# angelvillar96/STLPose

Measured on AMD Instinct MI355X. Metric: images/sec/GPU HRNet-W32 384x288 train step; PCKh@0.5 parity, higher is better.
Workload: dtype f16/bf16; 1 GPU; HRNet-W32 384x288 bs=32/GPU train step (fwd+MSE+bwd+Adam), random-init weights; global_batch=32, parallelism=dp1

## Files before the change

### stlpose_amd/csrc/wgrad.hip

```cpp
#include <type_traits>
#include "common.cuh"

#ifndef STL_DT
#define STL_DT 2
#endif

constexpr int WG_MAXG = STL_WGRAD_GROUP_MAX;
struct WgK {
    stl_wgrad p;
    stl_wgrad_io io[WG_MAXG];
    int ng;
    int dbg;
    int tiles_c, npt, HR, HC, HP, PI, pad, taps;
    int psg, psh;
    int off_cg, off_ch, off_g, off_h;
    float r_TW, r_HC, r_tc, r_vp, r_PI;
    unsigned long long m_tc, m_vp, m_PI;
    int xmap, units, gy, gz;
};

int stl_wgrad_backend_bf16(bool wide, const WgK& k, dim3 grid, size_t lds, hipStream_t st);
int stl_wgrad_backend_f32(bool wide, const WgK& k, dim3 grid, size_t lds, hipStream_t st);

namespace {

#include "conv_common.inc"

#ifdef STL_STAMPS
#include "../../include/stlpose_hip_debug.h"
__device__ long long g_wstamps[16];
__device__ long long g_wstamps2[64];
#define WSTAMP(i)                                                                                   \
    do {                                                                                            \
        if (k.dbg && blockIdx.x == 0 && blockIdx.y == 0 && blockIdx.z == 0 && threadIdx.x == 0) g_wstamps[i] = wall_clock64(); \
    } while (0)
#define WSTAMP2(i)                                                                                  \
    do {                                                                                            \
        if (k.dbg && blockIdx.x == 0 && blockIdx.y == 0 && blockIdx.z == 0 && threadIdx.x == 0 && (i) < 64) g_wstamps2[i] = wall_clock64(); \
    } while (0)
#else
#define WSTAMP(i) do {} while (0)
#define WSTAMP2(i) do {} while (0)
#endif

__device__ __forceinline__ int mad24_vsv(int a, int b_uniform, int c) {
    int r;
    asm("v_mad_i32_i24 %0, %1, %2, %3" : "=v"(r) : "v"(a), "s"(b_uniform), "v"(c));
    return r;
}

__device__ __forceinline__ int sdiv(int n, unsigned long long m) { return (int)(((unsigned long long)(uint32_t)n * m) >> 32); }


struct WgBlock { int member, bsplit, cy, cz; bool live; };
__device__ __forceinline__ WgBlock wg_block(const WgK& k) {
    WgBlock b;
    if (!k.xmap) {
        b.member = __builtin_amdgcn_readfirstlane(blockIdx.x / k.p.nsplit);
        b.bsplit = blockIdx.x - b.member * k.p.nsplit, b.cy = blockIdx.y, b.cz = blockIdx.z, b.live = true;
        return b;
    }
    const int nc = k.gy * k.gz, xcd = blockIdx.x & 7, j = blockIdx.x >> 3;
    const int ju = __builtin_amdgcn_readfirstlane(j / nc), chunk = j - ju * nc, unit = ju * 8 + xcd;
    b.live = unit < k.units;
    b.member = __builtin_amdgcn_readfirstlane(unit / k.p.nsplit), b.bsplit = unit - b.member * k.p.nsplit;
    b.cy = __builtin_amdgcn_readfirstlane(chunk / k.gz), b.cz = chunk - b.cy * k.gz;
    return b;
}


__device__ __forceinline__ int krow16(int g, int i, int lane) { return 16 * (g >> 1) + 8 * i + 4 * (g & 1) + ((lane & 15) >> 2); }

template <typename T>
__device__ __forceinline__ V16 frag_tr(const char* base, const int* rowoff, int colbyte, int lane);
template <>
__device__ __forceinline__ V16 frag_tr<__bf16>(const char* base, const int* rowoff, int colbyte, int lane) {
    V16 v;
#pragma unroll
    for (int h = 0; h < 2; ++h) {
        const char* ptr = base + rowoff[h] + colbyte + (lane & 3) * 8;
        s16x4 r = __builtin_amdgcn_ds_read_tr16_b64_v4i16(
            (__attribute__((address_space(3))) s16x4*)(uintptr_t)(uint32_t)(uintptr_t)ptr);
        const uint64_t bits = __builtin_bit_cast(uint64_t, r);
        v.w[2 * h] = (uint32_t)bits;
        v.w[2 * h + 1] = (uint32_t)(bits >> 32);
    }
    return v;
}
template <>
__device__ __forceinline__ V16 frag_tr<float>(const char* base, const int* rowoff, int colbyte, int lane) {
    V16 v;
#pragma unroll
    for (int s = 0; s < 4; ++s)
        v.w[s] = *reinterpret_cast<const uint32_t*>(base + rowoff[s] + colbyte + (lane & 15) * 4);
    return v;
}

template <typename T>
__device__ __forceinline__ V16 frag_at(const uint32_t* addr, int off);
template <>
__device__ __forceinline__ V16 frag_at<__bf16>(const uint32_t* addr, int off) {
    V16 v;
#pragma unroll
    for (int h = 0; h < 2; ++h) {
        s16x4 r = __builtin_amdgcn_ds_read_tr16_b64_v4i16((__attribute__((address_space(3))) s16x4*)(uintptr_t)(addr[h] + off));
        const uint64_t bits = __builtin_bit_cast(uint64_t, r);
        v.w[2 * h] = (uint32_t)bits;
        v.w[2 * h + 1] = (uint32_t)(bits >> 32);
    }
    return v;
}
template <>
__device__ __forceinline__ V16 frag_at<float>(const uint32_t* addr, int off) {
    V16 v;
#pragma unroll
    for (int s = 0; s < 4; ++s) v.w[s] = *(const __attribute__((address_space(3))) uint32_t*)(uintptr_t)(addr[s] + off);
    return v;
}

template <typename T, int KS, int NVH, bool GQ, int TPX, int OCC, int NW, typename TY = T, int CH = 32, int NSET = 2>
__global__ __launch_bounds__(64 * NW, OCC) void wgrad_kernel(const WgK k) {
    extern __shared__ __attribute__((aligned(16))) char smem[];
    constexpr int KV = ET<T>::KV, TAPS = KS * KS;
    constexpr int KSTEP = 4 * KV;
    constexpr int NR = sizeof(T) == 2 ? 2 : 4;
    constexpr int VPX = CH / KV;
    constexpr int NT = 64 * NW;
    constexpr int NVG = TPX * VPX / NT;
    static_assert(NVG >= 1 && NVG * NT == TPX * VPX, "g staging slots must tile the block");
    constexpr int QW = CH / 16, WPG = QW * QW;
    static_assert((CH == 32 || CH == 64) && NW % WPG == 0 && (NSET == 1 || NSET == 2), "channel tile / wave count");
    constexpr int NTG = NW / WPG;
    constexpr int TPG = (TAPS + NTG - 1) / NTG;
    constexpr int PS = CH * (int)sizeof(T) + (sizeof(T) == 2 ? 32 : 16);
    constexpr int NKT = TPX / KSTEP;
    const stl_wgrad& p = k.p;
    const WgBlock wb = wg_block(k);
    if (!wb.live) return;
    const int member = wb.member, bsplit = wb.bsplit;
    const stl_wgrad_io& io = k.io[member];
    const int tid = threadIdx.x, lane = tid & 63, wave = tid >> 6, g = lane >> 4;
    const int mt = (wave % WPG) / QW, nt = wave % QW, tg = wave / WPG;
    const int co0 = wb.cy * CH, ci0 = wb.cz * CH;
    WSTAMP(0);
    float* cgc = reinterpret_cast<float*>(smem + k.off_cg);
    float* chc = reinterpret_cast<float*>(smem + k.off_ch);
    char* sG = smem + k.off_g;
    char* sH = smem + k.off_h;

    const int tilepx = p.TH * p.TW;
    const int vpitch = p.Ho + 1;
    const int hrow = k.HC * PS;

    int g_yx[NVG];
    const int g_part = tid % VPX;
#pragma unroll
    for (int i = 0; i < NVG; ++i) {
        const int m = (tid + i * NT) / VPX;
        g_yx[i] = -1;
        if (m < tilepx) {
            const int ty = fdiv(m, k.r_TW);
            g_yx[i] = (ty << 16) | (m - ty * p.TW);
        }
    }
    int h_rc[NVH];
#pragma unroll
    for (int i = 0; i < NVH; ++i) {
        const int v = tid + i * NT;
        h_rc[i] = -1;
        if (v < k.HP * VPX) {
            const int hp = v / VPX, hr = fdiv(hp, k.r_HC);
            h_rc[i] = (hr << 16) | (hp - hr * k.HC);
        }
    }
    const bool g_chok = (co0 + g_part * KV) < p.Co, h_chok = (ci0 + g_part * KV) < p.Ci;

    const uint32_t lterm = sizeof(T) == 2 ? (lane & 3) * 8 : (lane & 15) * 4;
    uint32_t gaw[NR], hbw[NKT][NR];
#pragma unroll
    for (int i = 0; i < NR; ++i) {
        const int c = sizeof(T) == 2 ? krow16(g, i, lane) : 4 * g + i;
        gaw[i] = (uint32_t)(uintptr_t)sG + c * PS + lterm + mt * 16 * (int)sizeof(T);
#pragma unroll
        for (int s = 0; s < NKT; ++s) {
            int m = s * KSTEP + c;
            if (m >= tilepx) m = 0;
            const int ty = fdiv(m, k.r_TW), tx = m - ty * p.TW;
            hbw[s][i] = (uint32_t)(uintptr_t)sH + ((ty * p.stride) * k.HC + tx * p.stride) * PS + lterm + nt * 16 * (int)sizeof(T);
        }
    }

    V16 rgv[NSET][NVG], rgq[NSET][GQ ? NVG : 1], rhv[NSET][NVH];
    uint32_t okm[NSET] = {};

    const int g_cbytes = p.Co * (int)sizeof(T), h_cbytes = p.Ci * (int)sizeof(T);
    const int g_wrap = -p.Wo * g_cbytes, h_wrap = (p.Hi - k.PI) * p.Wi * h_cbytes;
    const int n_vp = -vpitch, n_PI = -k.PI;
    uint32_t g_lo[NVG], h_lo[NVH], slot_ok = 0;
#pragma unroll
    for (int i = 0; i < NVG; ++i) {
        g_lo[i] = (uint32_t)(((g_yx[i] >> 16) * p.Wo + (g_yx[i] & 0xffff)) * g_cbytes + (co0 + g_part * KV) * (int)sizeof(T));
        if (g_yx[i] >= 0 && g_chok) slot_ok |= 1u << i;
    }
#pragma unroll
    for (int i = 0; i < NVH; ++i) {
        h_lo[i] = (uint32_t)(((h_rc[i] >> 16) * p.Wi + (h_rc[i] & 0xffff)) * h_cbytes + (ci0 + g_part * KV) * (int)sizeof(T));
        if (h_rc[i] >= 0 && h_chok) slot_ok |= 1u << (NVG + i);
    }
    auto tile_offsets = [&](int t, uint32_t* go, uint32_t* ho) __attribute__((always_inline)) -> uint32_t {
        const int tr = sdiv(t, k.m_tc), tc = t - tr * k.tiles_c;
        const int vr0 = tr * p.TH, c0 = tc * p.TW;
        const int gb0 = sdiv(vr0, k.m_vp), gy0 = vr0 - gb0 * vpitch;
        const uint32_t g_t = (uint32_t)(((vr0 - gb0) * p.Wo + c0) * g_cbytes);
        uint32_t ok = 0;
#pragma unroll
        for (int i = 0; i < NVG; ++i) {
            const int oy0 = gy0 + (g_yx[i] >> 16), c = c0 + (g_yx[i] & 0xffff);
            const int wr_ = fdiv(oy0 < 0 ? 0 : oy0, k.r_vp);
            const int oy = mad24_vsv(wr_, n_vp, oy0);
            const bool in = ((slot_ok >> i) & 1u) & (gb0 + wr_ < p.B) & (oy < p.Ho) & (c < p.Wo);
            go[i] = in ? (uint32_t)mad24_vsv(wr_, g_wrap, (int)(g_t + g_lo[i])) : 0u;
            ok |= in ? 1u << i : 0u;
        }
        const int vrs = vr0 * p.stride, cb = c0 * p.stride - k.pad;
        const int hb0 = sdiv(vrs, k.m_PI), hy0 = vrs - hb0 * k.PI - k.pad;
        const uint32_t h_t = (uint32_t)(((hb0 * p.Hi + hy0) * p.Wi + cb) * h_cbytes);
#pragma unroll
        for (int i = 0; i < NVH; ++i) {
            const int iy0 = hy0 + (h_rc[i] >> 16), ix = cb + (h_rc[i] & 0xffff);
            const int wr_ = fdiv(iy0 < 0 ? 0 : iy0, k.r_PI);
            const int iy = mad24_vsv(wr_, n_PI, iy0);
            const bool in = ((slot_ok >> (NVG + i)) & 1u) & (iy0 >= 0) & (ix >= 0) & (ix < p.Wi) & (hb0 + wr_ < p.B) & (iy < p.Hi);
            ho[i] = in ? (uint32_t)mad24_vsv(wr_, h_wrap, (int)(h_t + h_lo[i])) : 0u;
            ok |= in ? 1u << (NVG + i) : 0u;
        }
        return ok;
    };
    auto load_set = [&](auto SET, const uint32_t* go, const uint32_t* ho, uint32_t ok) __attribute__((always_inline)) {
        constexpr int S = decltype(SET)::value;
#pragma unroll
        for (int i = 0; i < NVG; ++i) {
            rgv[S][i] = ldg16((const char*)io.g.x + go[i]);
            if (GQ) rgq[S][i] = ldg16((const char*)io.g.y + go[i]);
        }
#pragma unroll
        for (int i = 0; i < NVH; ++i) rhv[S][i] = ldg16((const char*)io.h.x + ho[i]);
        okm[S] = ok;
    };
    auto fetch = [&](auto SET, int t) __attribute__((always_inline)) {
        uint32_t go[NVG], ho[NVH];
        const uint32_t ok = tile_offsets(t, go, ho);
        load_set(SET, go, ho, ok);
    };
    const float relu_lo = io.h.relu ? 0.f : -INFINITY;
    auto write_lds = [&](auto SET) __attribute__((always_inline)) {
        constexpr int S = decltype(SET)::value;
        const int cl = g_part * KV;
#pragma unroll
        for (int i = 0; i < NVG; ++i) {
            V16 val = rgv[S][i];
            if (GQ) val = xform_bnbwd<T, TY>(val, rgq[S][i], cgc + cl, cgc + CH + cl, cgc + 2 * CH + cl);
            mask16(val, (okm[S] >> i) & 1u);
            const int v = tid + i * NT;
            *reinterpret_cast<V16*>(sG + (v / VPX) * PS + g_part * 16) = val;
        }
#pragma unroll
        for (int i = 0; i < NVH; ++i) {
            V16 val = rhv[S][i];
            if (io.h.mode == STL_SRC_BN) val = xform_bn<T, TY>(val, chc + cl, chc + CH + cl, relu_lo);
            else val = xform_cvt<T, TY>(val);
            mask16(val, (okm[S] >> (NVG + i)) & 1u);
            const int v = tid + i * NT;
            if (h_rc[i] >= 0) *reinterpret_cast<V16*>(sH + (v / VPX) * PS + g_part * 16) = val;
        }
    };

    f32x4 acc[TPG];
#pragma unroll
    for (int t = 0; t < TPG; ++t) acc[t] = f32x4{0.f, 0.f, 0.f, 0.f};

    auto mfma_taps = [&](auto TAP0, auto NTAP) __attribute__((always_inline)) {
        constexpr int T0 = decltype(TAP0)::value, NTP = decltype(NTAP)::value;
        constexpr int NJ = NKT * NTP, PF = NTP >= 4 ? (CH == 64 ? 4 : 6) : 2;
        uint32_t ga[NR], hb[NKT][NR];
#pragma unroll
        for (int i = 0; i < NR; ++i) {
            ga[i] = gaw[i];
            asm volatile("" : "+v"(ga[i]));
#pragma unroll
            for (int s = 0; s < NKT; ++s) {
                hb[s][i] = hbw[s][i];
                asm volatile("" : "+v"(hb[s][i]));
            }
        }
        V16 aq[2], bq[PF];
        auto bfrag = [&](int j) __attribute__((always_inline)) {
            const int s = j / NTP, tap = T0 + j % NTP;
            uint32_t ad[NR];
#pragma unroll
            for (int i = 0; i < NR; ++i) ad[i] = hb[s][i] + (tap / KS) * hrow;
            return frag_at<T>(ad, (tap % KS) * PS);
        };
        aq[0] = frag_at<T>(ga, 0);
#pragma unroll
        for (int j = 0; j < PF - 1 && j < NJ; ++j) bq[j] = bfrag(j);
#pragma unroll
        for (int j = 0; j < NJ; ++j) {
            const int s = j / NTP, jt = j % NTP;
            if (jt == 0 && s + 1 < NKT) aq[(s + 1) & 1] = frag_at<T>(ga, (s + 1) * KSTEP * PS);
            if (j + PF - 1 < NJ) bq[(j + PF - 1) % PF] = bfrag(j + PF - 1);
            mma16<T>(acc[jt], aq[s & 1], bq[j % PF]);
        }
    };
    auto mfma_tile = [&]() __attribute__((always_inline)) {
        if constexpr (NTG == 1) {
            mfma_taps(std::integral_constant<int, 0>{}, std::integral_constant<int, TAPS>{});
        } else {
            if (tg == 0) mfma_taps(std::integral_constant<int, 0>{}, std::integral_constant<int, TPG>{});
            else mfma_taps(std::integral_constant<int, TPG>{}, std::integral_constant<int, TAPS - TPG>{});
        }
    };

    const int step = p.nsplit;
    int t = bsplit;
    WSTAMP(1);
    SrcRaw raw;
    const int cidx = tid - (256 - 2 * CH);
    const bool cw = cidx >= 0 && cidx < 2 * CH, cg = cidx < CH;
    const int cch = cidx & (CH - 1);
    const bool cok = cw && (cg ? co0 + cch < p.Co : ci0 + cch < p.Ci);
    if (cok) {
        if (cg) src_raw_load(io.g, co0 + cch, p.Co, raw);
        else src_raw_load(io.h, ci0 + cch, p.Ci, raw);
    }
    constexpr std::integral_constant<int, 0> I0{};
    constexpr std::integral_constant<int, 1> I1{};
    if (t < k.npt) fetch(I0, t);
    if constexpr (NSET == 2) {
        if (t + step < k.npt) fetch(I1, t + step);
    }
    WSTAMP(2);
    if (cw) {
        float a = 0.f, b = 0.f, cc = 0.f;
        if (cok) {
            if (cg) src_raw_finish(io.g, raw, a, b, cc);
            else src_raw_finish(io.h, raw, a, b, cc);
        }
        if (cg) cgc[cch] = a, cgc[CH + cch] = b, cgc[2 * CH + cch] = cc;
        else chc[cch] = a, chc[CH + cch] = b;
    }
    __syncthreads();
    WSTAMP(3);
    bool first = true;
    [[maybe_unused]] int dbg_i = 0;
    auto body = [&](auto SET) __attribute__((always_inline)) {
        WSTAMP2(4 * dbg_i);
        write_lds(SET);
        __syncthreads();
        WSTAMP2(4 * dbg_i + 1);
        if (first) WSTAMP(4);
        if (t + NSET * step < k.npt) fetch(SET, t + NSET * step);
        WSTAMP2(4 * dbg_i + 2);
        mfma_tile();
        __syncthreads();
        WSTAMP2(4 * dbg_i + 3);
#ifdef STL_STAMPS
        ++dbg_i;
#endif
        if (first) WSTAMP(5);
        first = false;
        t += step;
    };
    while (t < k.npt) {
        body(I0);
        if constexpr (NSET == 2) {
            if (t >= k.npt) break;
            body(I1);
        }
    }
    WSTAMP(6);
    {
        float* slab = io.partial + (size_t)bsplit * p.Co * TAPS * p.Ci;
        const int ci = ci0 + nt * 16 + (lane & 15), co = co0 + mt * 16 + 4 * g;
        const int tap0 = tg * TPG;
        float* dst = slab + ((size_t)co * TAPS + tap0) * p.Ci + ci;
        if (ci < p.Ci) {
#pragma unroll
            for (int jt = 0; jt < TPG; ++jt)
#pragma unroll
                for (int r = 0; r < 4; ++r)
                    if (tap0 + jt < TAPS && co + r < p.Co) dst[((size_t)r * TAPS + jt) * p.Ci] = acc[jt][r];
        }
    }
    WSTAMP(8);
}


template <typename T, typename TY, int KS, int NVH, bool GQ, int TPX = 128, int NW = 4, int CH = 32>
int launch(const WgK& k, dim3 grid, size_t lds, hipStream_t st) {
    constexpr int OCC = NW == 16 ? 4 : ((NVH * NW <= 24 && TPX == 128 && sizeof(T) == 2) ? 2 : 1);
    constexpr int NSET = CH == 64 ? 1 : 2;
    static bool attr_done = false;
    if (!attr_done) {
        (void)hipFuncSetAttribute(reinterpret_cast<const void*>(&wgrad_kernel<T, KS, NVH, GQ, TPX, OCC, NW, TY, CH, NSET>),
                                  hipFuncAttributeMaxDynamicSharedMemorySize, 160 * 1024);
        attr_done = true;
    }
    STL_LAUNCH((wgrad_kernel<T, KS, NVH, GQ, TPX, OCC, NW, TY, CH, NSET>), grid, dim3(64 * NW), lds, st, k);
    static char nbuf[160];
    static const char* nm = stl_kname<T>(nbuf, "wgrad_kernel", {KS, NVH, GQ, TPX, OCC, NW, stl_code<TY>(), CH});
    stl_note_kernel(nm, true);
    STL_LAUNCH_CHECK("conv_wgrad");
    return 0;
}


template <typename T, int KS, int NVH, bool GQ, int TPX, typename TY = T>
__global__ __launch_bounds__(256) void wgrad64_kernel(const WgK k) {
    static_assert(sizeof(T) == 2, "bf16 only");
    extern __shared__ __attribute__((aligned(16))) char smem[];
    constexpr int KV = 8, TAPS = KS * KS, KSTEP = 32, NR = 2;
    constexpr int VPX = 8;
    constexpr int NVG = TPX * VPX / 256;
    constexpr int NKS = TPX / KSTEP;
    const stl_wgrad& p = k.p;
    const WgBlock wb = wg_block(k);
    if (!wb.live) return;
    const int member = wb.member, bsplit = wb.bsplit;
    const stl_wgrad_io& io = k.io[member];
    const int tid = threadIdx.x, lane = tid & 63, wave = tid >> 6, g = lane >> 4;
    const int wm = wave >> 1, wn = wave & 1;
    const int co0 = wb.cy * 64, ci0 = wb.cz * 64;
    float* cgc = reinterpret_cast<float*>(smem + k.off_cg);
    float* chc = reinterpret_cast<float*>(smem + k.off_ch);
    char* sG = smem + k.off_g;
    char* sH = smem + k.off_h;
    WSTAMP(0);

    const int tilepx = p.TH * p.TW;
    const int vpitch = p.Ho + 1;
    const int nks = (tilepx + KSTEP - 1) / KSTEP;

    int g_yx[NVG];
    const int g_part = tid % VPX;
#pragma unroll
    for (int i = 0; i < NVG; ++i) {
        const int m = (tid + i * 256) / VPX;
        g_yx[i] = -1;
        if (m < tilepx) {
            const int ty = fdiv(m, k.r_TW);
            g_yx[i] = (ty << 16) | (m - ty * p.TW);
        }
    }
    int h_rc[NVH];
#pragma unroll
    for (int i = 0; i < NVH; ++i) {
        const int v = tid + i * 256;
        h_rc[i] = -1;
        if (v < k.HP * VPX) {
            const int hp = v / VPX, hr = fdiv(hp, k.r_HC);
            h_rc[i] = (hr << 16) | (hp - hr * k.HC);
        }
    }
    const bool g_chok = (co0 + g_part * KV) < p.Co, h_chok = (ci0 + g_part * KV) < p.Ci;

    int rg0[NR], rh[NKS][NR];
#pragma unroll
    for (int i = 0; i < NR; ++i) rg0[i] = krow16(g, i, lane) * k.psg;
#pragma unroll
    for (int s = 0; s < NKS; ++s)
#pragma unroll
        for (int i = 0; i < NR; ++i) {
            int m = s * KSTEP + krow16(g, i, lane);
            if (m >= tilepx) m = 0;
            const int ty = fdiv(m, k.r_TW), tx = m - ty * p.TW;
            rh[s][i] = ((ty * p.stride) * k.HC + tx * p.stride) * k.psh;
        }

    V16 rgv[NVG], rgq[GQ ? NVG : 1], rhv[NVH];
    int g_go[NVG], h_go[NVH];

    auto setup = [&](int t) {
        const int tr = fdiv(t, k.r_tc), tc = t - tr * k.tiles_c;
        const int vr0 = tr * p.TH, c0 = tc * p.TW;
        const int gb0 = fdiv(vr0, k.r_vp), gy0 = vr0 - gb0 * vpitch;
#pragma unroll
        for (int i = 0; i < NVG; ++i) {
            g_go[i] = -1;
            if (g_yx[i] >= 0 && g_chok) {
                int oy = gy0 + (g_yx[i] >> 16), b = gb0;
                const int c = c0 + (g_yx[i] & 0xffff);
                { const int wr_ = fdiv(oy, k.r_vp); oy -= wr_ * vpitch, b += wr_; }
                if (b < p.B && oy < p.Ho && c < p.Wo) g_go[i] = ((b * p.Ho + oy) * p.Wo + c) * p.Co + co0 + g_part * KV;
            }
        }
        const int vrs = vr0 * p.stride, cb = c0 * p.stride - k.pad;
        const int hb0 = fdiv(vrs, k.r_PI), hy0 = vrs - hb0 * k.PI - k.pad;
#pragma unroll
        for (int i = 0; i < NVH; ++i) {
            h_go[i] = -1;
            if (h_rc[i] >= 0 && h_chok) {
                int iy = hy0 + (h_rc[i] >> 16), b = hb0;
                const int ix = cb + (h_rc[i] & 0xffff);
                if (iy >= 0 && ix >= 0 && ix < p.Wi) {
                    { const int wr_ = fdiv(iy, k.r_PI); iy -= wr_ * k.PI, b += wr_; }
                    if (b < p.B && iy < p.Hi) h_go[i] = ((b * p.Hi + iy) * p.Wi + ix) * p.Ci + ci0 + g_part * KV;
                }
            }
        }
    };
    auto issue = [&](bool en) {
#pragma unroll
        for (int i = 0; i < NVG; ++i) {
            const size_t off = (en && g_go[i] >= 0) ? (size_t)g_go[i] : 0;
            rgv[i] = ldg16((const char*)io.g.x + off * sizeof(T));
            if (GQ) rgq[i] = ldg16((const char*)io.g.y + off * sizeof(T));
        }
#pragma unroll
        for (int i = 0; i < NVH; ++i) {
            const size_t off = (en && h_go[i] >= 0) ? (size_t)h_go[i] : 0;
            rhv[i] = ldg16((const char*)io.h.x + off * sizeof(T));
        }
    };
    const float relu_lo = io.h.relu ? 0.f : -INFINITY;
    auto write_lds = [&]() {
        const int cl = g_part * KV;
#pragma unroll
        for (int i = 0; i < NVG; ++i) {
            V16 val = rgv[i];
            if (GQ) val = xform_bnbwd<T, TY>(val, rgq[i], cgc + cl, cgc + 64 + cl, cgc + 128 + cl);
            mask16(val, g_go[i] >= 0);
            const int v = tid + i * 256;
            *reinterpret_cast<V16*>(sG + (v / VPX) * k.psg + g_part * 16) = val;
        }
#pragma unroll
        for (int i = 0; i < NVH; ++i) {
            if (h_rc[i] < 0) continue;
            V16 val = rhv[i];
            if (io.h.mode == STL_SRC_BN) val = xform_bn<T, TY>(val, chc + cl, chc + 64 + cl, relu_lo);
            else val = xform_cvt<T, TY>(val);
            mask16(val, h_go[i] >= 0);
            const int v = tid + i * 256;
            *reinterpret_cast<V16*>(sH + (v / VPX) * k.psh + g_part * 16) = val;
        }
    };

    f32x4 acc[2][2][TAPS];
#pragma unroll
    for (int a = 0; a < 2; ++a)
#pragma unroll
        for (int b = 0; b < 2; ++b)
#pragma unroll
            for (int t = 0; t < TAPS; ++t) acc[a][b][t] = f32x4{0.f, 0.f, 0.f, 0.f};

    int t = bsplit;
    bool have = t < k.npt;
    WSTAMP(1);
    SrcRaw raw;
    const bool cw = wave >= 2, cg = wave == 3;
    const bool cok = cw && (cg ? co0 + lane < p.Co : ci0 + lane < p.Ci);
    if (cok) {
        if (cg) src_raw_load(io.g, co0 + lane, p.Co, raw);
        else src_raw_load(io.h, ci0 + lane, p.Ci, raw);
    }
    if (have) setup(t);
    issue(have);
    WSTAMP(2);
    if (cw) {
        float a = 0.f, b = 0.f, cc = 0.f;
        if (cok) {
            if (cg) src_raw_finish(io.g, raw, a, b, cc);
            else src_raw_finish(io.h, raw, a, b, cc);
        }
        if (cg) cgc[lane] = a, cgc[64 + lane] = b, cgc[128 + lane] = cc;
        else chc[lane] = a, chc[64 + lane] = b;
    }
    __syncthreads();
    WSTAMP(3);
    bool first = true;

    const int acol = (wm * 32) * (int)sizeof(T), bcol = (wn * 32) * (int)sizeof(T);
    while (have) {
        write_lds();
        __syncthreads();
        if (first) WSTAMP(4);
        const int tn = t + p.nsplit;
        const bool have_n = tn < k.npt;
        if (have_n) setup(tn);
        issue(have_n);
#pragma unroll
        for (int s = 0; s < NKS; ++s) {
            if (s < nks) {
                int rg[NR];
#pragma unroll
                for (int i = 0; i < NR; ++i) rg[i] = rg0[i] + s * KSTEP * k.psg;
                V16 a[2];
#pragma unroll
                for (int mt = 0; mt < 2; ++mt) a[mt] = frag_tr<T>(sG, rg, acol + mt * 16 * (int)sizeof(T), lane);
#pragma unroll
                for (int tap = 0; tap < TAPS; ++tap) {
                    const int toff = ((tap / KS) * k.HC + (tap % KS)) * k.psh;
#pragma unroll
                    for (int nt = 0; nt < 2; ++nt) {
                        const V16 b = frag_tr<T>(sH + toff, rh[s], bcol + nt * 16 * (int)sizeof(T), lane);
#pragma unroll
                        for (int mt = 0; mt < 2; ++mt) mma16<T>(acc[mt][nt][tap], a[mt], b);
                    }
                }
            }
        }
        __syncthreads();
        if (first) WSTAMP(5);
        first = false;
        t = tn, have = have_n;
    }
    WSTAMP(6);
    {
        float* slab = io.partial + (size_t)bsplit * p.Co * TAPS * p.Ci;
#pragma unroll
        for (int mt = 0; mt < 2; ++mt)
#pragma unroll
            for (int nt = 0; nt < 2; ++nt) {
                const int co = co0 + wm * 32 + mt * 16 + 4 * g, ci = ci0 + wn * 32 + nt * 16 + (lane & 15);
                float* dst = slab + (size_t)co * TAPS * p.Ci + ci;
                const bool ciok = ci < p.Ci;
#pragma unroll
                for (int tap = 0; tap < TAPS; ++tap)
#pragma unroll
                    for (int r = 0; r < 4; ++r)
                        if (ciok && co + r < p.Co) dst[((size_t)r * TAPS + tap) * p.Ci] = acc[mt][nt][tap][r];
            }
    }
    WSTAMP(8);
}

template <typename T, typename TY, int KS, int NVH, bool GQ, int TPX>
int launch64(const WgK& k, dim3 grid, size_t lds, hipStream_t st) {
    static bool attr_done = false;
    if (!attr_done) {
        (void)hipFuncSetAttribute(reinterpret_cast<const void*>(&wgrad64_kernel<T, KS, NVH, GQ, TPX, TY>),
                                  hipFuncAttributeMaxDynamicSharedMemorySize, 160 * 1024);
        attr_done = true;
    }
    STL_LAUNCH((wgrad64_kernel<T, KS, NVH, GQ, TPX, TY>), grid, dim3(256), lds, st, k);
    static char nbuf[160];
    static const char* nm = stl_kname<T>(nbuf, "wgrad64_kernel", {KS, NVH, GQ, TPX, stl_code<TY>()});
    stl_note_kernel(nm, true);
    STL_LAUNCH_CHECK("conv_wgrad64");
    return 0;
}

#if STL_DT != 0
template <typename TY>
int dispatch64(const WgK& k, dim3 grid, size_t lds, hipStream_t st) {
    const int nvh = ceil_div(k.HP * 8, 256);
    const bool gq = k.p.g.mode == STL_SRC_BNBWD;
    if (k.p.TH * k.p.TW <= 128 && nvh <= 6) return gq ? launch64<__bf16, TY, 1, 6, true, 128>(k, grid, lds, st) : launch64<__bf16, TY, 1, 6, false, 128>(k, grid, lds, st);
    return stl_set_error("wgrad64: halo of %d pixels is too large for a %d-pixel tile", k.HP, k.p.TH * k.p.TW);
}
#endif

dim3 wg_grid(WgK& k, int units, int gy, int gz) {
    const int xcd_env = getenv("STL_WGRAD_XCD") ? atoi(getenv("STL_WGRAD_XCD")) : 1;
    k.units = units, k.gy = gy, k.gz = gz;
    k.xmap = xcd_env && gy * gz > 1;
    if (!k.xmap) return dim3(units, gy, gz);
    return dim3(8 * ceil_div(units, 8) * gy * gz, 1, 1);
}

static bool wgrad_c64_3x3(const stl_wgrad& p) {
    const char* e = getenv("STL_WGRAD_C64");
    return !(e && atoi(e) == 0) && p.dtype == STL_BF16 && p.ks == 3 && p.stride == 1 && p.Co >= 64 && p.Ci >= 64;
}

int wgrad_chunk(const stl_wgrad& p) {
    if (wgrad_c64_3x3(p)) return 64;
    return (p.dtype == STL_BF16 && p.ks == 1 && p.stride == 1 && p.Co >= 64 && p.Ci >= 64) ? 64 : 32;
}

template <typename T, typename TY, int KS>
int dispatch(const WgK& k, dim3 grid, size_t lds, hipStream_t st) {
    {
        const int64_t gpx = (int64_t)k.p.B * k.p.Ho * k.p.Wo, hpx = (int64_t)k.p.B * k.p.Hi * k.p.Wi;
        const bool small = gpx * k.p.Co * (int64_t)sizeof(T) < ((int64_t)1 << 32) && hpx * k.p.Ci * (int64_t)sizeof(T) < ((int64_t)1 << 32) &&
                           (int64_t)k.p.Wo * k.p.Co * (int64_t)sizeof(T) < (1 << 23) &&
                           (int64_t)(k.PI > k.p.Hi ? k.PI - k.p.Hi : k.p.Hi - k.PI) * k.p.Wi * k.p.Ci * (int64_t)sizeof(T) < (1 << 23) &&
                           k.PI < (1 << 12) && k.tiles_c < (1 << 12) && (int64_t)k.npt * k.p.TH * k.p.stride < (1 << 20);
        STL_CHECK(small, "wgrad: tensors of 4 GB or more, rows beyond 8 MB or more than 4095 rows / tile columns are not addressable");
    }
    const int vpx = 32 / ET<T>::KV;
    const int nvh = ceil_div(k.HP * vpx, 256);
    const bool gq = k.p.g.mode == STL_SRC_BNBWD;
    STL_CHECK(k.p.TH * k.p.TW <= 128, "wgrad: tiles of more than 128 pixels are not supported");
    if constexpr (KS == 3 && sizeof(T) == 2) {
        if (k.p.ks == 3 && wgrad_c64_3x3(k.p)) {
            const int nvh16 = ceil_div(k.HP * 8, 1024);
            if (nvh16 <= 2) return gq ? launch<T, TY, KS, 2, true, 128, 16, 64>(k, grid, lds, st) : launch<T, TY, KS, 2, false, 128, 16, 64>(k, grid, lds, st);
            if (nvh16 <= 3) return gq ? launch<T, TY, KS, 3, true, 128, 16, 64>(k, grid, lds, st) : launch<T, TY, KS, 3, false, 128, 16, 64>(k, grid, lds, st);
            return stl_set_error("wgrad: halo of %d pixels is too large for the 64-channel 3x3 kernel; shrink the tile", k.HP);
        }
    }
    if constexpr (KS == 3) {
        const int nvh8 = ceil_div(k.HP * vpx, 512);
        if (nvh8 <= 2) return gq ? launch<T, TY, KS, 2, true, 128, 8>(k, grid, lds, st) : launch<T, TY, KS, 2, false, 128, 8>(k, grid, lds, st);
        if (nvh8 <= 3) return gq ? launch<T, TY, KS, 3, true, 128, 8>(k, grid, lds, st) : launch<T, TY, KS, 3, false, 128, 8>(k, grid, lds, st);
        if (nvh8 <= 5) return gq ? launch<T, TY, KS, 5, true, 128, 8>(k, grid, lds, st) : launch<T, TY, KS, 5, false, 128, 8>(k, grid, lds, st);
        if (nvh8 <= 9) return gq ? launch<T, TY, KS, 9, true, 128, 8>(k, grid, lds, st) : launch<T, TY, KS, 9, false, 128, 8>(k, grid, lds, st);
        return stl_set_error("wgrad: halo of %d pixels is too large for the 3x3 kernel; shrink the tile", k.HP);
    }
    if (nvh <= 3) return gq ? launch<T, TY, KS, 3, true>(k, grid, lds, st) : launch<T, TY, KS, 3, false>(k, grid, lds, st);
    if (nvh <= 6) return gq ? launch<T, TY, KS, 6, true>(k, grid, lds, st) : launch<T, TY, KS, 6, false>(k, grid, lds, st);
    if (nvh <= 9) return gq ? launch<T, TY, KS, 9, true>(k, grid, lds, st) : launch<T, TY, KS, 9, false>(k, grid, lds, st);
    if (nvh <= 18) return gq ? launch<T, TY, KS, 18, true>(k, grid, lds, st) : launch<T, TY, KS, 18, false>(k, grid, lds, st);
    return stl_set_error("wgrad: halo of %d pixels needs %d staging vectors per thread (max 18); shrink the tile", k.HP, nvh);
}

}

#if STL_DT != 0
int stl_wgrad_backend_bf16(bool wide, const WgK& k, dim3 grid, size_t lds, hipStream_t st) {
    if (k.p.ydtype == STL_F16) {
        if (wide) return dispatch64<f16>(k, grid, lds, st);
        return k.p.ks == 3 ? dispatch<__bf16, f16, 3>(k, grid, lds, st) : dispatch<__bf16, f16, 1>(k, grid, lds, st);
    }
    if (wide) return dispatch64<__bf16>(k, grid, lds, st);
    return k.p.ks == 3 ? dispatch<__bf16, __bf16, 3>(k, grid, lds, st) : dispatch<__bf16, __bf16, 1>(k, grid, lds, st);
}
#endif
#if STL_DT != 1
int stl_wgrad_backend_f32(bool wide, const WgK& k, dim3 grid, size_t lds, hipStream_t st) {
    if (wide) return stl_set_error("wgrad: the 64 x 64-channel variant is bf16 only");
    return k.p.ks == 3 ? dispatch<float, float, 3>(k, grid, lds, st) : dispatch<float, float, 1>(k, grid, lds, st);
}
#endif

#if STL_DT != 0
#ifdef STL_STAMPS
extern "C" int stl_debug_wgrad_stamps2(long long* host64) {
    return hipMemcpyFromSymbol(host64, HIP_SYMBOL(g_wstamps2), 64 * sizeof(long long)) == hipSuccess ? 0 : stl_set_error("stamps: copy failed");
}
extern "C" int stl_debug_wgrad_stamps(long long* host16) {
    return hipMemcpyFromSymbol(host16, HIP_SYMBOL(g_wstamps), 16 * sizeof(long long)) == hipSuccess ? 0 : stl_set_error("stamps: copy failed");
}
#endif

extern "C" int stl_wgrad_chunk(const stl_wgrad* pp) { return wgrad_chunk(*pp); }

static int wgrad_run(const stl_wgrad* const* ps, int ng, void* stream);

extern "C" int stl_conv_wgrad(const stl_wgrad* pp, void* stream) { return wgrad_run(&pp, 1, stream); }

extern "C" int stl_conv_wgrad_group(const stl_wgrad_group* grp, void* stream) {
    STL_CHECK(grp && grp->n >= 1 && grp->n <= WG_MAXG, "wgrad_group: 1..%d members", WG_MAXG);
    const stl_wgrad& a = *grp->p[0];
    for (int i = 1; i < grp->n; ++i) {
        const stl_wgrad& b = *grp->p[i];
        STL_CHECK(b.dtype == a.dtype && b.B == a.B && b.Hi == a.Hi && b.Wi == a.Wi && b.Ci == a.Ci && b.Ho == a.Ho && b.Wo == a.Wo &&
                      b.Co == a.Co && b.ks == a.ks && b.stride == a.stride && b.TH == a.TH && b.TW == a.TW && b.nsplit == a.nsplit &&
                      b.g.mode == a.g.mode,
                  "wgrad_group: member %d differs from member 0 in geometry, tile, nsplit or gradient source mode", i);
    }
    return wgrad_run(grp->p, grp->n, stream);
}

static int wgrad_run(const stl_wgrad* const* ps, int ng, void* stream) {
    const stl_wgrad& p = *ps[0];
  for (int i_ = 0; i_ < ng; ++i_) {
    const stl_wgrad& p = *ps[i_];
    STL_CHECK(p.dtype == STL_F32 || p.dtype == STL_BF16, "wgrad: bad dtype (gradients are fp32 or bf16)");
    STL_CHECK(p.ydtype == 0 || p.ydtype == p.dtype || (p.dtype == STL_BF16 && p.ydtype == STL_F16), "wgrad: ydtype %d does not go with dtype %d", p.ydtype, p.dtype);
    STL_CHECK(p.ydtype == ps[0]->ydtype, "wgrad_group: members differ in ydtype");
    STL_CHECK(p.ks == 1 || p.ks == 3, "wgrad: ks must be 1 or 3");
    STL_CHECK(p.stride == 1 || p.stride == 2, "wgrad: stride must be 1 or 2");
    const int kv = p.dtype == STL_BF16 ? 8 : 4;
    STL_CHECK(p.Ci % kv == 0 && p.Co % kv == 0, "wgrad: Ci=%d / Co=%d must be multiples of %d", p.Ci, p.Co, kv);
    STL_CHECK(p.TH >= 1 && p.TW >= 1 && p.TH * p.TW <= 128, "wgrad: tile exceeds 128 pixels");
    STL_CHECK((int64_t)p.B * p.Hi * p.Wi * p.Ci < (1ll << 31) && (int64_t)p.B * p.Ho * p.Wo * p.Co < (1ll << 31),
              "wgrad: tensors of 2^31 or more elements are not supported");
    const int pad = p.ks == 3 ? 1 : 0;
    STL_CHECK((p.Hi + 2 * pad - p.ks) / p.stride + 1 == p.Ho && (p.Wi + 2 * pad - p.ks) / p.stride + 1 == p.Wo,
              "wgrad: output %dx%d inconsistent with input %dx%d", p.Ho, p.Wo, p.Hi, p.Wi);
    STL_CHECK(p.h.x && p.g.x && p.partial && p.nsplit >= 1, "wgrad: null pointer / nsplit");
    STL_CHECK(p.h.mode == STL_SRC_PLAIN || p.h.mode == STL_SRC_BN, "wgrad: h must be PLAIN or BN");
    STL_CHECK(p.g.mode == STL_SRC_PLAIN || p.g.mode == STL_SRC_BNBWD, "wgrad: g must be PLAIN or BNBWD");
    STL_CHECK(p.g.mode != STL_SRC_BNBWD || (p.g.y && p.g.stats && p.g.rstats && p.g.gamma), "wgrad: BNBWD source incomplete");
    STL_CHECK(p.h.mode != STL_SRC_BN || (p.h.gamma && p.h.beta && (p.h.stats || (p.h.rmean && p.h.rvar))), "wgrad: BN source incomplete");
  }
    const int pad = p.ks == 3 ? 1 : 0;
    WgK k;
    k.p = p;
    k.ng = ng;
    for (int i = 0; i < ng; ++i) k.io[i].h = ps[i]->h, k.io[i].g = ps[i]->g, k.io[i].partial = ps[i]->partial;
    k.dbg = getenv("STL_CONV_STAMPS") ? 1 : 0;
    k.taps = p.ks * p.ks;
    k.pad = pad;
    k.PI = p.stride * (p.Ho + 1);
    k.HR = (p.TH - 1) * p.stride + p.ks;
    k.HC = (p.TW - 1) * p.stride + p.ks;
    k.HP = k.HR * k.HC;
    k.tiles_c = ceil_div(p.Wo, p.TW);
    k.npt = ceil_div(p.B * (p.Ho + 1), p.TH) * k.tiles_c;
    k.r_TW = 1.0f / p.TW, k.r_HC = 1.0f / k.HC, k.r_tc = 1.0f / k.tiles_c, k.r_vp = 1.0f / (p.Ho + 1), k.r_PI = 1.0f / k.PI;
    const unsigned long long two32 = 1ull << 32;
    k.m_tc = (two32 + k.tiles_c - 1) / k.tiles_c, k.m_vp = (two32 + p.Ho) / (p.Ho + 1), k.m_PI = (two32 + k.PI - 1) / k.PI;
    STL_CHECK((int64_t)k.npt < (1 << 21) && (int64_t)p.B * k.PI < (1 << 21), "wgrad: too many tiles");
    hipStream_t st = (hipStream_t)stream;
    if (wgrad_c64_3x3(p)) {
        k.psg = k.psh = 64 * 2 + 32;
        k.off_cg = 0, k.off_ch = 3 * 64 * 4, k.off_g = 2048;
        k.off_h = k.off_g + 128 * k.psg;
        const size_t ldsw = (size_t)k.off_h + (size_t)k.HP * k.psh;
        STL_CHECK(ldsw <= 160 * 1024, "wgrad: tile needs %zu B of LDS (>160 KiB)", ldsw);
        STL_CHECK(p.nsplit <= k.npt || p.nsplit == 1, "wgrad: nsplit %d > tiles %d", p.nsplit, k.npt);
        dim3 gridw = wg_grid(k, p.nsplit * ng, ceil_div(p.Co, 64), ceil_div(p.Ci, 64));
        return stl_wgrad_backend_bf16(false, k, gridw, ldsw, st);
    }
    if (wgrad_chunk(p) == 64) {
        k.psg = k.psh = 160;
        k.off_cg = 0, k.off_ch = 3 * 64 * 4, k.off_g = 2048;
        k.off_h = k.off_g + 128 * k.psg;
        const size_t lds64 = (size_t)k.off_h + (size_t)k.HP * k.psh;
        STL_CHECK(lds64 <= 160 * 1024, "wgrad64: tile needs %zu B of LDS (>160 KiB)", lds64);
        STL_CHECK(p.nsplit <= k.npt || p.nsplit == 1, "wgrad: nsplit %d > tiles %d", p.nsplit, k.npt);
        dim3 grid64 = wg_grid(k, p.nsplit * ng, ceil_div(p.Co, 64), ceil_div(p.Ci, 64));
        return stl_wgrad_backend_bf16(true, k, grid64, lds64, st);
    }
    const int esz = p.dtype == STL_BF16 ? 2 : 4;
    k.psg = k.psh = 32 * esz + (esz == 2 ? 32 : 16);
    k.off_cg = 0;
    k.off_ch = 3 * 32 * 4;
    k.off_g = 1024;
    int szG = 128 * k.psg;
    int szH = k.HP * k.psh;
    k.off_h = k.off_g + szG;
    size_t lds = (size_t)k.off_h + szH;
    STL_CHECK(lds <= 160 * 1024, "wgrad: tile needs %zu B of LDS (>160 KiB)", lds);
    STL_CHECK(p.nsplit <= k.npt || p.nsplit == 1, "wgrad: nsplit %d > tiles %d", p.nsplit, k.npt);
    dim3 grid = wg_grid(k, p.nsplit * ng, ceil_div(p.Co, 32), ceil_div(p.Ci, 32));
    return p.dtype == STL_BF16 ? stl_wgrad_backend_bf16(false, k, grid, lds, st) : stl_wgrad_backend_f32(false, k, grid, lds, st);
}
#endif
```

Before: 2466 images/sec.

## Double-buffer LDS images in 64-channel 3x3 wgrad kernel to overlap staging with MFMA

Adds a two-image LDS ping-pong path for the 16-wave 64-channel 3x3 bf16 weight-gradient kernel. The next tile is written to the alternate LDS image while the current image feeds the MFMA loop, which removes one of the two barriers per tile. The cost is twice the LDS footprint per block, which may reduce occupancy, and the path is only used when the halo fits in two vectors. It can be disabled with an environment variable.

```diff
diff --git a/stlpose_amd/csrc/wgrad.hip b/stlpose_amd/csrc/wgrad.hip
--- a/stlpose_amd/csrc/wgrad.hip
+++ b/stlpose_amd/csrc/wgrad.hip
@@ -14,6 +14,7 @@
     int tiles_c, npt, HR, HC, HP, PI, pad, taps;
     int psg, psh;
     int off_cg, off_ch, off_g, off_h;
+    int img;
     float r_TW, r_HC, r_tc, r_vp, r_PI;
     unsigned long long m_tc, m_vp, m_PI;
     int xmap, units, gy, gz;
@@ -118,7 +119,7 @@
     return v;
 }
 
-template <typename T, int KS, int NVH, bool GQ, int TPX, int OCC, int NW, typename TY = T, int CH = 32, int NSET = 2>
+template <typename T, int KS, int NVH, bool GQ, int TPX, int OCC, int NW, typename TY = T, int NIMG = 1, int CH = 32, int NSET = 2>
 __global__ __launch_bounds__(64 * NW, OCC) void wgrad_kernel(const WgK k) {
     extern __shared__ __attribute__((aligned(16))) char smem[];
     constexpr int KV = ET<T>::KV, TAPS = KS * KS;
@@ -130,6 +131,7 @@
     static_assert(NVG >= 1 && NVG * NT == TPX * VPX, "g staging slots must tile the block");
     constexpr int QW = CH / 16, WPG = QW * QW;
     static_assert((CH == 32 || CH == 64) && NW % WPG == 0 && (NSET == 1 || NSET == 2), "channel tile / wave count");
+    static_assert(NIMG == 1 || (NIMG == 2 && NSET == 1 && CH == 64 && NW == 16), "two LDS images: the 16-wave block only");
     constexpr int NTG = NW / WPG;
     constexpr int TPG = (TAPS + NTG - 1) / NTG;
     constexpr int PS = CH * (int)sizeof(T) + (sizeof(T) == 2 ? 32 : 16);
@@ -253,9 +255,11 @@
         load_set(SET, go, ho, ok);
     };
     const float relu_lo = io.h.relu ? 0.f : -INFINITY;
-    auto write_lds = [&](auto SET) __attribute__((always_inline)) {
+    auto write_lds = [&](auto SET, int img) __attribute__((always_inline)) {
         constexpr int S = decltype(SET)::value;
         const int cl = g_part * KV;
+        char* const sG = smem + k.off_g + img;
+        char* const sH = smem + k.off_h + img;
 #pragma unroll
         for (int i = 0; i < NVG; ++i) {
             V16 val = rgv[S][i];
@@ -279,17 +283,17 @@
 #pragma unroll
     for (int t = 0; t < TPG; ++t) acc[t] = f32x4{0.f, 0.f, 0.f, 0.f};
 
-    auto mfma_taps = [&](auto TAP0, auto NTAP) __attribute__((always_inline)) {
+    auto mfma_taps = [&](auto TAP0, auto NTAP, int img) __attribute__((always_inline)) {
         constexpr int T0 = decltype(TAP0)::value, NTP = decltype(NTAP)::value;
         constexpr int NJ = NKT * NTP, PF = NTP >= 4 ? (CH == 64 ? 4 : 6) : 2;
         uint32_t ga[NR], hb[NKT][NR];
 #pragma unroll
         for (int i = 0; i < NR; ++i) {
-            ga[i] = gaw[i];
+            ga[i] = gaw[i] + img;
             asm volatile("" : "+v"(ga[i]));
 #pragma unroll
             for (int s = 0; s < NKT; ++s) {
-                hb[s][i] = hbw[s][i];
+                hb[s][i] = hbw[s][i] + img;
                 asm volatile("" : "+v"(hb[s][i]));
             }
         }
@@ -312,12 +316,12 @@
             mma16<T>(acc[jt], aq[s & 1], bq[j % PF]);
         }
     };
-    auto mfma_tile = [&]() __attribute__((always_inline)) {
+    auto mfma_tile = [&](int img) __attribute__((always_inline)) {
         if constexpr (NTG == 1) {
-            mfma_taps(std::integral_constant<int, 0>{}, std::integral_constant<int, TAPS>{});
+            mfma_taps(std::integral_constant<int, 0>{}, std::integral_constant<int, TAPS>{}, img);
         } else {
-            if (tg == 0) mfma_taps(std::integral_constant<int, 0>{}, std::integral_constant<int, TPG>{});
-            else mfma_taps(std::integral_constant<int, TPG>{}, std::integral_constant<int, TAPS - TPG>{});
+            if (tg == 0) mfma_taps(std::integral_constant<int, 0>{}, std::integral_constant<int, TPG>{}, img);
+            else mfma_taps(std::integral_constant<int, TPG>{}, std::integral_constant<int, TAPS - TPG>{}, img);
         }
     };
 
@@ -355,13 +359,13 @@
     [[maybe_unused]] int dbg_i = 0;
     auto body = [&](auto SET) __attribute__((always_inline)) {
         WSTAMP2(4 * dbg_i);
-        write_lds(SET);
+        write_lds(SET, 0);
         __syncthreads();
         WSTAMP2(4 * dbg_i + 1);
         if (first) WSTAMP(4);
         if (t + NSET * step < k.npt) fetch(SET, t + NSET * step);
         WSTAMP2(4 * dbg_i + 2);
-        mfma_tile();
+        mfma_tile(0);
         __syncthreads();
         WSTAMP2(4 * dbg_i + 3);
 #ifdef STL_STAMPS
@@ -371,11 +375,45 @@
         first = false;
         t += step;
     };
-    while (t < k.npt) {
-        body(I0);
-        if constexpr (NSET == 2) {
-            if (t >= k.npt) break;
-            body(I1);
+    auto body2 = [&](int cur) __attribute__((always_inline)) {
+        int img_r = cur, img_w = k.img - cur;
+        asm volatile("" : "+s"(img_r), "+s"(img_w));
+        WSTAMP2(4 * dbg_i);
+        if (t + step < k.npt) {
+            write_lds(I0, img_w);
+            __builtin_amdgcn_sched_barrier(0);
+            WSTAMP2(4 * dbg_i + 1);
+            if (t + 2 * step < k.npt) fetch(I0, t + 2 * step);
+        } else {
+            WSTAMP2(4 * dbg_i + 1);
+        }
+        WSTAMP2(4 * dbg_i + 2);
+        __builtin_amdgcn_sched_barrier(0);
+        mfma_tile(img_r);
+        __syncthreads();
+        WSTAMP2(4 * dbg_i + 3);
+#ifdef STL_STAMPS
+        ++dbg_i;
+#endif
+        if (first) WSTAMP(5);
+        first = false;
+        t += step;
+    };
+    if constexpr (NIMG == 2) {
+        if (t < k.npt) {
+            write_lds(I0, 0);
+            if (t + step < k.npt) fetch(I0, t + step);
+            __syncthreads();
+            WSTAMP(4);
+        }
+        for (int cur = 0; t < k.npt; cur = k.img - cur) body2(cur);
+    } else {
+        while (t < k.npt) {
+            body(I0);
+            if constexpr (NSET == 2) {
+                if (t >= k.npt) break;
+                body(I1);
+            }
         }
     }
     WSTAMP(6);
@@ -396,19 +434,19 @@
 }
 
 
-template <typename T, typename TY, int KS, int NVH, bool GQ, int TPX = 128, int NW = 4, int CH = 32>
+template <typename T, typename TY, int KS, int NVH, bool GQ, int TPX = 128, int NW = 4, int CH = 32, int NIMG = 1>
 int launch(const WgK& k, dim3 grid, size_t lds, hipStream_t st) {
     constexpr int OCC = NW == 16 ? 4 : ((NVH * NW <= 24 && TPX == 128 && sizeof(T) == 2) ? 2 : 1);
     constexpr int NSET = CH == 64 ? 1 : 2;
     static bool attr_done = false;
     if (!attr_done) {
-        (void)hipFuncSetAttribute(reinterpret_cast<const void*>(&wgrad_kernel<T, KS, NVH, GQ, TPX, OCC, NW, TY, CH, NSET>),
+        (void)hipFuncSetAttribute(reinterpret_cast<const void*>(&wgrad_kernel<T, KS, NVH, GQ, TPX, OCC, NW, TY, NIMG, CH, NSET>),
                                   hipFuncAttributeMaxDynamicSharedMemorySize, 160 * 1024);
         attr_done = true;
     }
-    STL_LAUNCH((wgrad_kernel<T, KS, NVH, GQ, TPX, OCC, NW, TY, CH, NSET>), grid, dim3(64 * NW), lds, st, k);
+    STL_LAUNCH((wgrad_kernel<T, KS, NVH, GQ, TPX, OCC, NW, TY, NIMG, CH, NSET>), grid, dim3(64 * NW), lds, st, k);
     static char nbuf[160];
-    static const char* nm = stl_kname<T>(nbuf, "wgrad_kernel", {KS, NVH, GQ, TPX, OCC, NW, stl_code<TY>(), CH});
+    static const char* nm = stl_kname<T>(nbuf, "wgrad_kernel", {KS, NVH, GQ, TPX, OCC, NW, stl_code<TY>(), NIMG, CH});
     stl_note_kernel(nm, true);
     STL_LAUNCH_CHECK("conv_wgrad");
     return 0;
@@ -673,6 +711,13 @@
     return !(e && atoi(e) == 0) && p.dtype == STL_BF16 && p.ks == 3 && p.stride == 1 && p.Co >= 64 && p.Ci >= 64;
 }
 
+static int wgrad_c64_image_bytes(int HP, int ps) {
+    const char* e = getenv("STL_WGRAD_IMAGES");
+    if (e && atoi(e) == 1) return 0;
+    const int img = ((128 + HP) * ps + 31) & ~31;
+    return (HP * 8 <= 2 * 1024 && 2048 + 2 * (size_t)img <= 160 * 1024) ? img : 0;
+}
+
 int wgrad_chunk(const stl_wgrad& p) {
     if (wgrad_c64_3x3(p)) return 64;
     return (p.dtype == STL_BF16 && p.ks == 1 && p.stride == 1 && p.Co >= 64 && p.Ci >= 64) ? 64 : 32;
@@ -695,6 +740,8 @@
     if constexpr (KS == 3 && sizeof(T) == 2) {
         if (k.p.ks == 3 && wgrad_c64_3x3(k.p)) {
             const int nvh16 = ceil_div(k.HP * 8, 1024);
+            if (nvh16 <= 2 && k.img) return gq ? launch<T, TY, KS, 2, true, 128, 16, 64, 2>(k, grid, lds, st) : launch<T, TY, KS, 2, false, 128, 16, 64, 2>(k, grid, lds, st);
+            STL_CHECK(!k.img, "wgrad: two LDS images exist for the two-halo-vector form only");
             if (nvh16 <= 2) return gq ? launch<T, TY, KS, 2, true, 128, 16, 64>(k, grid, lds, st) : launch<T, TY, KS, 2, false, 128, 16, 64>(k, grid, lds, st);
             if (nvh16 <= 3) return gq ? launch<T, TY, KS, 3, true, 128, 16, 64>(k, grid, lds, st) : launch<T, TY, KS, 3, false, 128, 16, 64>(k, grid, lds, st);
             return stl_set_error("wgrad: halo of %d pixels is too large for the 64-channel 3x3 kernel; shrink the tile", k.HP);
@@ -789,6 +836,7 @@
     const int pad = p.ks == 3 ? 1 : 0;
     WgK k;
     k.p = p;
+    k.img = 0;
     k.ng = ng;
     for (int i = 0; i < ng; ++i) k.io[i].h = ps[i]->h, k.io[i].g = ps[i]->g, k.io[i].partial = ps[i]->partial;
     k.dbg = getenv("STL_CONV_STAMPS") ? 1 : 0;
@@ -809,7 +857,8 @@
         k.psg = k.psh = 64 * 2 + 32;
         k.off_cg = 0, k.off_ch = 3 * 64 * 4, k.off_g = 2048;
         k.off_h = k.off_g + 128 * k.psg;
-        const size_t ldsw = (size_t)k.off_h + (size_t)k.HP * k.psh;
+        k.img = wgrad_c64_image_bytes(k.HP, k.psg);
+        const size_t ldsw = k.img ? (size_t)k.off_g + 2 * (size_t)k.img : (size_t)k.off_h + (size_t)k.HP * k.psh;
         STL_CHECK(ldsw <= 160 * 1024, "wgrad: tile needs %zu B of LDS (>160 KiB)", ldsw);
         STL_CHECK(p.nsplit <= k.npt || p.nsplit == 1, "wgrad: nsplit %d > tiles %d", p.nsplit, k.npt);
         dim3 gridw = wg_grid(k, p.nsplit * ng, ceil_div(p.Co, 64), ceil_div(p.Ci, 64));
```

New measurement: 2483 images/sec, median of 6. Within noise of the previous version (+0.7%).
